# stephane-caron/qpmpc

Measured on AMD Instinct MI355X. Metric: MPC QP builds+solves/sec (batched), higher is better.
Workload: dtype f64

## Files before the change

qpmpc_amd/csrc/mpcqp_quad.hip:

```cpp
#include <hip/hip_runtime.h>
#include <math.h>
#include <stdint.h>
#include <type_traits>

#include "mpcqp.h"
#include "mpcqp_internal.h"
#include "mpcqp_quad_common.h"

namespace mpcqp {

namespace quad {

constexpr int MMAX = 32;
constexpr int MK = 2;

}

using namespace quad;

template <int NX, bool ORD, int WPB, bool SLIM, bool MODEL = false, bool GEN = false>
__global__ void __launch_bounds__(64 * WPB, SLIM ? 2 : 1)
    mpcqp_quad_kernel(const double *__restrict__ gA, const double *__restrict__ gB, const double *__restrict__ gC,
                      const double *__restrict__ ge, const double *__restrict__ gx0, const double *__restrict__ ggoal,
                      const double *__restrict__ gtgt, double *__restrict__ oU, double *__restrict__ olam, int32_t *__restrict__ ostatus,
                      int32_t *__restrict__ oiters, const KernelArgs ka, const int64_t batch)
{
    using T = double;
    extern __shared__ __attribute__((aligned(16))) unsigned char smem_raw[];
    {
        const int64_t b0 = ka.A.batch_stride, b1 = ka.B.batch_stride, b2 = ka.C.batch_stride, b3 = ka.e.batch_stride,
                      b4 = ka.x0.batch_stride, b5 = ka.goal.batch_stride;
        const int64_t s0 = ka.A.step_stride, s1 = ka.B.step_stride, s2 = ka.C.step_stride, s3 = ka.e.step_stride;
        asm volatile("" ::"s"(b0), "s"(b1), "s"(b2), "s"(b3), "s"(b4), "s"(b5), "s"(s0), "s"(s1), "s"(s2), "s"(s3), "s"(ka.N), "s"(ka.nu),
                     "s"(ka.flags), "s"(ka.probe), "s"(gA), "s"(gB), "s"(gC), "s"(ge), "s"(gx0), "s"(ggoal), "s"(ka.n), "s"(ka.m),
                     "s"(batch));
    }
    const int lane = threadIdx.x & 63;
    const int wv = threadIdx.x >> 6;
    const int rb = lane & 48;
    const int l = lane & 15;
    int64_t prob = 4 * ((int64_t)blockIdx.x * WPB + wv) + (rb >> 4);
    const bool valid = prob < batch;
    prob = valid ? prob : batch - 1;
    if constexpr (ORD) {
        const int64_t o = ka.order[prob];
        prob = o < 0 ? 0 : (o >= batch ? batch - 1 : o);
    }
    using CV = Carve<SLIM>;
    constexpr int LDM = CV::LDM, PER = CV::PER;
    T *sm = (T *)smem_raw + (4 * wv + (rb >> 4)) * PER;
    const int n = ka.n, m = ka.m;
    const int row0 = l, row1 = l + NV;
    const bool isc0 = row0 < m, isc1 = row1 < m;
    const T INF = HUGE_VAL;
    constexpr int GS = 33;
    T *Gimg = sm + CV::OFF_M, *Ml = sm + CV::OFF_M;
    T *LTp = sm + CV::OFF_LT + (l * (31 - l)) / 2 - (l + 1);
    T *LTimg = sm + CV::OFF_LT, *Timg = sm + CV::OFF_T, *kAv = sm + CV::OFF_KA;
    int *actv = reinterpret_cast<int *>(sm + CV::OFF_ACT);

    long long *stamp = ka.probe ? (long long *)ka.probe + prob * 16 : nullptr;
    auto tick = [&](int slot) {
        if (stamp && l == 0 && valid) {
            stamp[slot] = (long long)__builtin_readcyclecounter();
            if (slot == 0 || slot == 6) stamp[slot ? 13 : 12] = (long long)__builtin_amdgcn_s_memrealtime();
        }
    };
    tick(0);

    T hval0, hval1;
    bool notpd = false;
    T RM0[NV], RM1[NV], RLt[NV];
    T wv_ = T(0);
    if constexpr (MODEL) {
        const T *model = gA;
        const ModelLayout ml = make_model_layout(ka.nx, ka.N, n, m);
        const int nxr = ka.nx, nT = ka.N * ka.nx;
        const T *x0 = gx0 + prob * ka.x0.batch_stride;
        const T *goal = ggoal ? ggoal + prob * ka.goal.batch_stride : nullptr;
        const T *tgt = gtgt ? gtgt + prob * ka.targets.batch_stride : nullptr;
        notpd = model[ml.total] != T(0);
        {
            T r0[NV], r1[NV];
            ld16(r0, model + ml.off_M + (size_t)(isc0 ? row0 : 0) * NV);
            ld16(r1, model + ml.off_M + (size_t)(isc1 ? row1 : 0) * NV);
            ld16(RLt, model + ml.off_LinvT + (size_t)l * NV);
#pragma unroll
            for (int k = 0; k < NV; ++k) {
                RM0[k] = isc0 ? r0[k] : T(0);
                RM1[k] = isc1 ? r1[k] : T(0);
            }
        }
        auto bound = [&](int row, bool isc) {
            if (!isc) return INF;
            const int mkr = ka.mk, kq = mkr == 2 ? row >> 1 : row / mkr;
            T hh = ge ? ge[prob * ka.e.batch_stride + kq * ka.e.step_stride + (row - kq * mkr)] : model[ml.off_e + row];
            for (int c = 0; c < nxr; ++c) hh -= model[ml.off_Hx + (size_t)row * nxr + c] * x0[c];
            return hh;
        };
        hval0 = bound(row0, isc0);
        hval1 = bound(row1, isc1);
        for (int c = 0; c < nxr; ++c) wv_ += model[ml.off_Wx + (size_t)l * nxr + c] * x0[c];
        if ((ka.flags & MPCQP_Q_TERMINAL) && goal)
            for (int c = 0; c < nxr; ++c) wv_ -= model[ml.off_Wg + (size_t)l * nxr + c] * goal[c];
        if ((ka.flags & MPCQP_Q_STAGE) && tgt)
            for (int j2 = 0; j2 < nT; ++j2) wv_ -= model[ml.off_Wt + (size_t)l * nT + j2] * tgt[j2];
        tick(1);
    } else {
    T Pr[NV];
    T qa;
    T g15a = T(0), g15b = T(0);
    {
        constexpr bool WIDE = GEN && NX > 6;
        const int nx = WIDE ? ka.nx : NX;
        const int nu = ka.nu, N = ka.N;
        constexpr int MKG = GEN ? 4 : MK;
        const int mk = GEN ? ka.mk : MK;
        auto stepof = [&](int row) { return mk == 2 ? row >> 1 : (mk == 1 ? row : (mk == 4 ? row >> 2 : row / 3)); };
        const T *A = gA + prob * ka.A.batch_stride;
        const T *B = gB + prob * ka.B.batch_stride;
        const bool hasC = !GEN || gC != nullptr;
        const T *Cm = hasC ? gC + prob * ka.C.batch_stride : A;
        const T *x0 = gx0 + prob * ka.x0.batch_stride;
        const T *goal = ggoal ? ggoal + prob * ka.goal.batch_stride : nullptr;
        const int sA = ka.A.step_stride ? nx * nx : 0, sB = ka.B.step_stride ? nx * nu : 0, sC = (hasC && ka.C.step_stride) ? mk * nx : 0;
        const bool termP = ka.flags & MPCQP_P_TERMINAL, termQ = (ka.flags & MPCQP_Q_TERMINAL) && goal;
        const T *Dm = (GEN && ka.D.ptr) ? (const T *)ka.D.ptr + prob * ka.D.batch_stride : nullptr;
        const T *tgt = (GEN && gtgt) ? gtgt + prob * ka.targets.batch_stride : nullptr;
        const int sD = (GEN && ka.D.step_stride) ? mk * nu : 0;
        const bool stageP = GEN && (ka.flags & MPCQP_P_STAGE), stageQ = GEN && (ka.flags & MPCQP_Q_STAGE) && tgt;
        constexpr int NAe = NX * NX, NEe = NAe + MKG * NX;
        const int NEr = hasC ? NAe + mk * NX : NAe;
        const bool col = (l < n);
        const int j = col ? (nu == 1 ? l : l / nu) : -1, ii = col ? l - j * nu : 0;
        const int64_t eb = prob * ka.e.batch_stride;
        const int kq0 = stepof(row0), kq1 = stepof(row1);
        const T eval0 = isc0 ? ge[eb + kq0 * ka.e.step_stride + (row0 - kq0 * mk)] : INF;
        const T eval1 = isc1 ? ge[eb + kq1 * ka.e.step_stride + (row1 - kq1 * mk)] : INF;
        const bool xl15 = (l == NV - 1);
        T v[NX], gref[NX], bcol[NX];
#pragma unroll
        for (int s = 0; s < NX; ++s) {
            v[s] = (xl15 && s < nx) ? x0[s < nx ? s : 0] : T(0);
            gref[s] = (termQ && s < nx) ? goal[s < nx ? s : 0] : T(0);
        }
#pragma unroll
        for (int r = 0; r < NX; ++r) bcol[r] = (col && r < nx) ? B[j * sB + (r < nx ? r : 0) * nu + ii] : T(0);
        T dcol[MKG], d15a = T(0), d15b = T(0), tg[NX];
#pragma unroll
        for (int u = 0; u < NX; ++u) tg[u] = T(0);
#pragma unroll
        for (int i2 = 0; i2 < MKG; ++i2) dcol[i2] = T(0);
        if constexpr (GEN) {
            if (Dm) {
#pragma unroll
                for (int i2 = 0; i2 < MKG; ++i2) dcol[i2] = (col && !xl15 && i2 < mk) ? Dm[j * sD + i2 * nu + ii] : T(0);
                if (n == NV) {
                    const int j15 = nu == 1 ? NV - 1 : (NV - 1) / nu, i15 = NV - 1 - j15 * nu;
                    d15a = (isc0 && kq0 == j15) ? Dm[j15 * sD + (row0 - kq0 * mk) * nu + i15] : T(0);
                    d15b = (isc1 && kq1 == j15) ? Dm[j15 * sD + (row1 - kq1 * mk) * nu + i15] : T(0);
                }
            }
            if (stageQ && !WIDE) {
#pragma unroll
                for (int u = 0; u < NX; ++u) tg[u] = (l + 16 * u < N * NX) ? tgt[l + 16 * u] : T(0);
            }
        }
        if constexpr (!WIDE) {
        constexpr int NOP = (NEe + 15) / 16;
        T op[NOP][NV];
        static_for<0, NOP>([&](auto rc) {
            constexpr int r = decltype(rc)::value;
            const int e = l + 16 * r;
            const bool ok = e < NEr;
            const T *p = (e < NAe) ? A + e : Cm + (ok ? e - NAe : 0);
            const int st = (e < NAe) ? sA : sC;
#pragma unroll
            for (int k = 0; k < NV; ++k) {
                const int kc = (k < N) ? k : N - 1;
                op[r][k] = p[kc * st];
            }
        });
        tick(8);
        const T wu = (T)ka.wu;
        qa = T(0);
#pragma unroll
        for (int b = 0; b < NV; ++b) Pr[b] = (l == b) ? (col ? wu : T(1)) : T(0);
        tick(9);
        auto mac = [&](auto idx, auto kc_, T &acc, T xx) {
            constexpr int IDX = decltype(idx)::value, K = decltype(kc_)::value;
            fmac_bcast<IDX % 16>(acc, op[IDX / 16][K], xx);
        };
        static_for<0, NV>([&](auto kk) {
            constexpr int k = decltype(kk)::value;
            if (k < N) {
                if constexpr (!GEN) {
                    T g[MK];
                    static_for<0, MK>([&](auto i2c) {
                        constexpr int i2 = decltype(i2c)::value;
                        T acc = T(0);
                        static_for<0, NX>([&](auto sc) {
                            constexpr int s2 = decltype(sc)::value;
                            mac(ic<NAe + i2 * NX + s2>{}, kk, acc, v[s2]);
                        });
                        g[i2] = acc;
                    });
#pragma unroll
                    for (int i2 = 0; i2 < MK; ++i2) Gimg[l * GS + k * MK + i2] = g[i2];
                } else {
                    static_for<0, MKG>([&](auto i2c) {
                        constexpr int i2 = decltype(i2c)::value;
                        if (i2 < mk) {
                            T acc = T(0);
                            if (hasC) {
                                static_for<0, NX>([&](auto sc) {
                                    constexpr int s2 = decltype(sc)::value;
                                    mac(ic<NAe + i2 * NX + s2>{}, kk, acc, v[s2]);
                                });
                            }
                            acc += (j == k) ? dcol[i2] : T(0);
                            Gimg[l * GS + k * mk + i2] = acc;
                        }
                    });
                }
                if constexpr (GEN && k >= 1) {
                    if (stageP || stageQ) {
                        const T wxs = (T)ka.wx;
                        static_for<0, NX>([&](auto sc) {
                            constexpr int s2 = decltype(sc)::value;
                            constexpr int te = k * NX + s2;
                            T src = xl15 ? T(0) : v[s2];
                            const T t = wxs * src;
                            if (stageQ) qa += t * (row_bcast<NV - 1>(v[s2]) - row_bcast<te % 16>(tg[te / 16]));
                            if (stageP) {
                                dpp_ready(src);
                                static_for<0, NV>([&](auto bc) { fmac_bcast<decltype(bc)::value>(Pr[decltype(bc)::value], src, t); });
                            }
                        });
                    }
                }
                const T hk = (j == k && !xl15) ? T(1) : T(0);
                T w[NX];
                static_for<0, NX>([&](auto rc) {
                    constexpr int r = decltype(rc)::value;
                    T acc = hk * bcol[r];
                    static_for<0, NX>([&](auto sc) {
                        constexpr int s2 = decltype(sc)::value;
                        mac(ic<r * NX + s2>{}, kk, acc, v[s2]);
                    });
                    w[r] = acc;
                });
#pragma unroll
                for (int r = 0; r < NX; ++r) v[r] = w[r];
            }
        });
        } else {
        tick(8);
        const T wu = (T)ka.wu;
        qa = T(0);
#pragma unroll
        for (int b = 0; b < NV; ++b) Pr[b] = (l == b) ? (col ? wu : T(1)) : T(0);
        tick(9);
        constexpr int NAw = NX * NX, NCw = 4 * NX, NEw = NAw + NCw + NX, NOPW = (NEw + 15) / 16;
        T opw[2][NOPW];
        auto fetch = [&](auto dc, int k) {
            constexpr int d = decltype(dc)::value;
            const int kc = k < N ? k : N - 1;
            static_for<0, NOPW>([&](auto rc) {
                constexpr int r = decltype(rc)::value;
                constexpr int e0 = 16 * r;
                const int e = e0 + l;
                T val;
                if constexpr (e0 < NAw) {
                    const int rr = e / NX, ss = e - rr * NX;
                    const bool ok = rr < nx && ss < nx;
                    val = A[kc * sA + (ok ? rr * nx + ss : 0)];
                    val = ok ? val : T(0);
                } else if constexpr (e0 < NAw + NCw) {
                    const int e2 = e - NAw, i2 = e2 / NX, ss = e2 - i2 * NX;
                    const bool ok = hasC && i2 < mk && ss < nx;
                    val = Cm[ok ? kc * sC + i2 * nx + ss : 0];
                    val = ok ? val : T(0);
                } else {
                    const int ss = e - NAw - NCw;
                    const bool ok = stageQ && ss < nx;
                    val = ok ? tgt[kc * nx + ss] : T(0);
                }
                opw[d][r] = val;
            });
        };
        fetch(ic<0>{}, 0);
        fetch(ic<1>{}, 1);
        const T wxs = (T)ka.wx;
        auto cstep = [&](auto dc, int k) {
            constexpr int d = decltype(dc)::value;
            static_for<0, NOPW>([&](auto rc) { dpp_ready(opw[d][decltype(rc)::value]); });
            static_for<0, 4>([&](auto i2c) {
                constexpr int i2 = decltype(i2c)::value;
                if (i2 < mk) {
                    T acc = T(0);
                    if (hasC) {
                        static_for<0, NX>([&](auto sc) {
                            constexpr int s2 = decltype(sc)::value, E = NAw + i2 * NX + s2;
                            fmac_bcast<E % 16>(acc, opw[d][E / 16], v[s2]);
                        });
                    }
                    acc += (j == k) ? dcol[i2] : T(0);
                    Gimg[l * GS + k * mk + i2] = acc;
                }
            });
            if (k >= 1 && (stageP || stageQ)) {
                static_for<0, NX>([&](auto sc) {
                    constexpr int s2 = decltype(sc)::value, E = NAw + NCw + s2;
                    T src = xl15 ? T(0) : v[s2];
                    const T t = wxs * src;
                    if (stageQ) qa += t * (row_bcast<NV - 1>(v[s2]) - row_bcast<E % 16>(opw[d][E / 16]));
                    if (stageP) {
                        dpp_ready(src);
                        static_for<0, NV>([&](auto bc) { fmac_bcast<decltype(bc)::value>(Pr[decltype(bc)::value], src, t); });
                    }
                });
            }
            const T hk = (j == k && !xl15) ? T(1) : T(0);
            T w[NX];
            static_for<0, NX>([&](auto rc) {
                constexpr int r = decltype(rc)::value;
                T acc = hk * bcol[r];
                static_for<0, NX>([&](auto sc) {
                    constexpr int s2 = decltype(sc)::value, E = r * NX + s2;
                    fmac_bcast<E % 16>(acc, opw[d][E / 16], v[s2]);
                });
                w[r] = acc;
            });
#pragma unroll
            for (int r = 0; r < NX; ++r) v[r] = w[r];
            fetch(dc, k + 2);
        };
        for (int k = 0; k < N; k += 2) {
            cstep(ic<0>{}, k);
            if (k + 1 < N) cstep(ic<1>{}, k + 1);
        }
        }
        tick(10);
        const T wt = (T)ka.wt;
        T x[NX];
#pragma unroll
        for (int s = 0; s < NX; ++s) {
            x[s] = row_bcast<NV - 1>(v[s]);
            v[s] = xl15 ? bcol[s] : v[s];
        }
#pragma unroll
        for (int s = 0; s < NX; ++s) {
            const T t = wt * v[s];
            if (termQ) qa += t * (x[s] - gref[s]);
            if (termP) {
                T src = v[s];
                dpp_ready(src);
                static_for<0, NV>([&](auto bc) { fmac_bcast<decltype(bc)::value>(Pr[decltype(bc)::value], src, t); });
            }
        }
        qa = col ? qa : T(0);
        tick(11);
        wave_sync();
        hval0 = isc0 ? eval0 - Gimg[(NV - 1) * GS + row0] : INF;
        hval1 = isc1 ? eval1 - Gimg[(NV - 1) * GS + row1] : INF;
        if constexpr (GEN) {
            g15a = d15a;
            g15b = d15b;
        }
    }
    tick(1);
    {
#pragma unroll
        for (int k = 0; k < NV; ++k) {
            RM0[k] = (isc0 && k < NV - 1) ? Gimg[k * GS + row0] : (GEN && k == NV - 1 ? g15a : T(0));
            RM1[k] = (isc1 && k < NV - 1) ? Gimg[k * GS + row1] : (GEN && k == NV - 1 ? g15b : T(0));
            RLt[k] = (l == k) ? T(1) : T(0);
        }
        static_for<0, NV>([&](auto jc) {
            constexpr int j = decltype(jc)::value;
            const T pij = Pr[j];
            const T piv = row_bcast<j>(pij);
            if (!(piv > T(0))) notpd = true;
            const T rinv = fast_rsqrt(piv);
            const T nt2 = -(pij * rinv * rinv);
            T nl = -(pij * rinv);
            RM0[j] *= rinv;
            RM1[j] *= rinv;
            RLt[j] *= rinv;
            const T wj = qa * rinv;
            wv_ = (l == j) ? wj : wv_;
            {
                T src = pij, wsrc = wj;
                asm volatile("s_nop 1" : "+v"(src), "+v"(nl), "+v"(wsrc) : "v"(RM0[j]), "v"(RM1[j]), "v"(RLt[j]));
                fmac_bcast<j>(qa, wsrc, nl);
                static_for<j + 1, NV>([&](auto kc) {
                    constexpr int k = decltype(kc)::value;
                    fmac_bcast<k>(Pr[k], src, nt2);
                    fmac_bcast<k>(RM0[k], nl, RM0[j]);
                    fmac_bcast<k>(RM1[k], nl, RM1[j]);
                    fmac_bcast<k>(RLt[k], nl, RLt[j]);
                });
            }
        });
        wave_sync();
    }
    }
    tick(2);
    tick(3);
    int status = MPCQP_MAX_ITER, iters = 0;
    T xsol = T(0);
    bool done = notpd;
    bool finished = notpd;
    if (notpd) status = MPCQP_NOT_PD;

    if (isc0) st16(Ml + row0 * LDM, RM0);
    if (isc1) st16(Ml + row1 * LDM, RM1);
    T ltd = T(0);
    if constexpr (SLIM) {
        static_for<0, NV>([&](auto kc) {
            constexpr int k = decltype(kc)::value;
            ltd = (l == k) ? RLt[k] : ltd;
            if (k > l) LTp[k] = RLt[k];
        });
    } else {
        st16(LTimg + l * NV, RLt);
    }
    const T y0 = -wv_;
    T s0, s1, invn0, invn1;
    {
        const T d0 = dot_bcast(wv_, RM0, hval0), d1 = dot_bcast(wv_, RM1, hval1);
        s0 = isc0 ? d0 : INF;
        s1 = isc1 ? d1 : INF;
        const T nn0 = dot16(RM0, RM0), nn1 = dot16(RM1, RM1);
        invn0 = (nn0 > T(0)) ? fast_rsqrt(nn0) : T(1);
        invn1 = (nn1 > T(0)) ? fast_rsqrt(nn1) : T(1);
    }
    const bool sel0 = isc0 && (hval0 < T(1e29)), sel1 = isc1 && (hval1 < T(1e29));
    const T tol = (T)ka.tol;
    const T tolh0 = tol + tol * fabs(hval0), tolh1 = tol + tol * fabs(hval1);
    const int max_iter = ka.max_iter;
    T RT[NV], RH[NV];
#pragma unroll
    for (int k = 0; k < NV; ++k) {
        RT[k] = T(0);
        RH[k] = (l == k) ? T(1) : T(0);
    }
    T lam = T(0);
    int myact = 0;
    bool occ = false;
    bool e0 = sel0, e1 = sel1;
    int nq = 0, p = 0, ldrop = 0;
    unsigned mask = 0;
    bool needp = true, dropping = false;
    T up = T(0);
    int fails = 0;
    T mp[NV];
    auto select = [&]() {
        const bool want = needp & !done & !dropping;
        const unsigned h0 = ~(unsigned)__double2hiint(s0 * invn0), h1 = ~(unsigned)__double2hiint(s1 * invn1);
        const bool v0 = want & e0 & (s0 < -tolh0), v1 = want & e1 & (s1 < -tolh1);
        const unsigned k0 = v0 ? ((h0 & ~31u) | (unsigned)row0) : 0xffffffffu;
        const unsigned k1 = v1 ? ((h1 & ~31u) | (unsigned)row1) : 0xffffffffu;
        const unsigned mkey = row_min(min(k0, k1));
        const bool none = want & (mkey == 0xffffffffu);
        const bool got = want & !none;
        done = done | none;
        status = none ? (int)MPCQP_SOLVED : status;
        p = got ? (int)(mkey & 31u) : p;
        up = got ? T(0) : up;
        needp = needp & !got;
    };
    auto update = [&](auto bc, auto ec, T zn, T cT, T cH) {
        static_for<decltype(bc)::value, decltype(ec)::value>([&](auto kc) {
            constexpr int k = decltype(kc)::value;
            fmac_bcast<k>(RT[k], zn, cT);
            fmac_bcast<k>(RH[k], zn, cH);
        });
    };
#ifndef QUAD_USPLIT
#define QUAD_USPLIT 8
#endif
    constexpr int USPLIT = QUAD_USPLIT;
    T zn = T(0), cT = T(0), cH = T(0);
    wave_sync();
    tick(4);
    for (;;) {
#include "mpcqp_quad_steady.h"
        if (general) for (;;) {
            dpp_ready(zn);
            update(ic<0>{}, ic<USPLIT>{}, zn, cT, cH);
            select();
            ld16(mp, Ml + p * LDM);
            update(ic<USPLIT>{}, ic<NV>{}, zn, cT, cH);
            cT = cH = T(0);
            if (__ballot(!done) == 0ull) break;
            const bool st = !done & !dropping;
            const bool drp = !done & dropping;
            const bool phi = p >= NV;
            const int pl = p & 15;
            const T hd = dot16(RH, mp);
            const T kd0 = dot_bcast(hd, RM0, T(0)), kd1 = dot_bcast(hd, RM1, T(0));
            T inv, t2;
            {
                const T kp = phi ? kd1 : kd0, sq = phi ? s1 : s0, iq = phi ? invn1 : invn0;
                const bool okf = kp * iq * iq > T(DEP_FAST);
                const T iv = fast_rcp(kp);
                inv = row_get(okf ? iv : T(-1), rb, pl);
                t2 = row_get(-sq * iv, rb, pl);
            }
            T rd = dot16(RT, mp);
            pin(rd);
            if (__ballot(st & !(inv > T(0))) != 0ull) {
                T z2 = hd * hd;
                z2 += dpp_mov<ROR8>(z2);
                z2 += dpp_mov<ROR4>(z2);
                z2 += dpp_mov<ROR2>(z2);
                z2 += dpp_mov<ROR1>(z2);
                z2 = row_bcast<0>(z2);
                const T sq = row_get(phi ? s1 : s0, rb, pl), iq = row_get(phi ? invn1 : invn0, rb, pl);
                const bool ok2 = (z2 * iq * iq > T(DEP)) & (z2 > T(0));
                const T iv2 = fast_rcp(z2);
                const bool nearp = !(inv > T(0));
                t2 = nearp ? -sq * iv2 : t2;
                inv = nearp ? (ok2 ? iv2 : T(0)) : inv;
            }
            const bool can_move = (nq < n) & (inv > T(0));
            inv = (can_move & st) ? inv : T(0);
            t2 = can_move ? t2 : INF;
            const int sl = (int)__builtin_ctz(~mask);
            const T r = (occ & st) ? rd : T(0);
            const bool blk = (r > T(0)) & (lam < t2 * r);
            if (__ballot(drp | (st & (!can_move | (iters >= max_iter) | blk))) == 0ull) {
                const T tt = st ? t2 : T(0);
                const bool isnew = st & (l == sl), isp = st & (l == pl);
                iters += st ? 1 : 0;
                zn = hd;
                cT = (l == sl) ? inv : -(r * inv);
                cH = -(hd * inv);
                s0 = fma(tt, kd0, s0);
                s1 = fma(tt, kd1, s1);
                T ln = fma(-tt, r, lam);
                ln = (occ & (ln < T(0))) ? T(0) : ln;
                lam = isnew ? up + tt : ln;
                myact = isnew ? p : myact;
                occ = occ | isnew;
                e0 = e0 & !(isp & !phi);
                e1 = e1 & !(isp & phi);
                mask |= st ? (1u << sl) : 0u;
                nq += st ? 1 : 0;
                needp = needp | st;
                continue;
            }
            bool stepping = st;
            {
                const bool lim = stepping & (iters >= max_iter);
                done = done | lim;
                finished = finished | lim;
                status = lim ? (int)MPCQP_MAX_ITER : status;
                stepping = stepping & !lim;
            }
            iters += stepping ? 1 : 0;
            const bool cand = occ & stepping & (r > T(0));
            T t1 = INF;
            int lq = 0;
            const unsigned long long bl = __ballot(stepping & blk);
            if (bl != 0ull) {
                const T ratio = cand ? lam * fast_rcp(r) : INF;
                unsigned hi, lo;
                ordered(ratio, hi, lo);
                hi = cand ? hi : 0xffffffffu;
                const unsigned mhi = row_min(hi);
                const unsigned k2 = (cand && hi == mhi) ? ((lo & ~31u) | (unsigned)l) : 0xffffffffu;
                const unsigned ml = row_min(k2);
                lq = (int)(ml & 15u);
                const T tl1 = row_get(ratio, rb, lq);
                const bool blocked = ((unsigned)(bl >> rb) & 0xffffu) != 0u;
                t1 = (blocked && mhi != 0xffffffffu) ? tl1 : INF;
            }
            T t = t1 < t2 ? t1 : t2;
            {
                const bool inf = stepping & !(t < INF);
                done = done | inf;
                finished = finished | inf;
                status = inf ? (int)MPCQP_INFEASIBLE : status;
                stepping = stepping & !inf;
            }
            t = stepping ? t : T(0);
            const bool full = stepping & (t2 <= t1);
            zn = hd;
            cT = full ? ((l == sl) ? inv : -(r * inv)) : T(0);
            cH = full ? -(hd * inv) : T(0);
            if (__ballot(drp) != 0ull) {
                T vv[NV];
                T vl = T(0);
                if constexpr (SLIM) {
#pragma unroll
                    for (int k = 0; k < NV; ++k) {
                        vv[k] = row_get(RT[k], rb, ldrop);
                        vl = (l == k) ? vv[k] : vl;
                    }
                } else {
                    ld16(vv, kAv);
                    vl = kAv[l];
                }
                const T tl = dot16(RT, vv);
                const T tld = row_get(tl, rb, ldrop);
                const T itl = fast_rcp(tld);
                if (drp) {
                    zn = vl;
                    cT = (l == ldrop) ? T(-1) : (occ ? -tl * itl : T(0));
                    cH = vl * itl;
                    if (l == ldrop) {
                        lam = T(0);
                        occ = false;
                    }
                    mask &= ~(1u << ldrop);
                    --nq;
                    dropping = false;
                }
            }
            if (stepping) {
                s0 = fma(t, kd0, s0);
                s1 = fma(t, kd1, s1);
                lam -= t * r;
                lam = (occ && lam < T(0)) ? T(0) : lam;
                up += t;
            }
            if (full) {
                if (l == sl) {
                    lam = up;
                    myact = p;
                    occ = true;
                }
                if (l == pl) {
                    e0 = e0 & phi;
                    e1 = e1 & !phi;
                }
                mask |= 1u << sl;
                ++nq;
                needp = true;
            }
            const bool partial = stepping & !full;
            if (__ballot(partial) != 0ull) {
                const int cl = row_get(myact, rb, lq);
                if constexpr (!SLIM) {
                    wave_sync();
                    if (partial && l == lq) st16(kAv, RT);
                }
                if (partial) {
                    if (l == (cl & 15)) {
                        e0 = (cl < NV) ? sel0 : e0;
                        e1 = (cl < NV) ? e1 : sel1;
                    }
                    dropping = true;
                    ldrop = lq;
                }
                if constexpr (!SLIM) wave_sync();
            }
        }
        tick(5);
        if (__ballot(!finished) == 0ull) break;
        int aa[NV];
        if constexpr (SLIM) {
            const int mine = occ ? myact : 0;
            static_for<0, NV>([&](auto ac) { aa[decltype(ac)::value] = __builtin_amdgcn_update_dpp(0, mine, 0x150 + decltype(ac)::value, 0xf, 0xf, false); });
        } else {
            actv[l] = occ ? myact : 0;
            wave_sync();
            const int4 *ap = reinterpret_cast<const int4 *>(actv);
#pragma unroll
            for (int q = 0; q < NV / 4; ++q) {
                const int4 t4 = ap[q];
                aa[4 * q] = t4.x;
                aa[4 * q + 1] = t4.y;
                aa[4 * q + 2] = t4.z;
                aa[4 * q + 3] = t4.w;
            }
        }
        auto ma_dot = [&](T cf) {
            T ma[NV];
#pragma unroll
            for (int a = 0; a < NV; ++a) ma[a] = Ml[aa[a] * LDM + l];
            return dot_bcast(cf, ma, T(0));
        };
        T fresh0, fresh1;
        auto slacks = [&](T yv) {
            const T f0 = dot_bcast(yv, RM0, T(0)), f1 = dot_bcast(yv, RM1, T(0));
            fresh0 = isc0 ? hval0 - f0 : INF;
            fresh1 = isc1 ? hval1 - f1 : INF;
        };
        auto of_act = [&](T x0v, T x1v) {
            const T a = row_get(x0v, rb, myact & 15), b = row_get(x1v, rb, myact & 15);
            return (myact < NV) ? a : b;
        };
        T y = y0 - ma_dot(occ ? lam : T(0));
        slacks(y);
        T rho = of_act(fresh0, fresh1);
        rho = occ ? rho : T(0);
        constexpr double REFTOL = 1e-11;
        const T hact = of_act(hval0, hval1);
        const bool needref = occ & !finished & !(fabs(rho) <= T(REFTOL) * (T(1) + fabs(hact)));
        const unsigned long long nr = __ballot(needref);
        if (nr != 0ull) {
            rho = (((unsigned)(nr >> rb) & 0xffffu) != 0u) ? rho : T(0);
            T uk = T(0);
            if constexpr (SLIM) {
                static_for<0, NV>([&](auto kc) {
                    constexpr int k = decltype(kc)::value;
                    T v = RT[k] * rho;
                    v += dpp_mov<ROR8>(v);
                    v += dpp_mov<ROR4>(v);
                    v += dpp_mov<ROR2>(v);
                    v += dpp_mov<ROR1>(v);
                    uk = (l == k) ? v : uk;
                });
            } else {
                st16(Timg + l * NV, RT);
                wave_sync();
                T tc[NV];
#pragma unroll
                for (int a = 0; a < NV; ++a) tc[a] = Timg[a * NV + l];
                uk = dot_bcast(rho, tc, T(0));
            }
            T dl = -dot_bcast(uk, RT, T(0));
            dl = occ ? dl : T(0);
            if (!finished) {
                const T lraw = lam + dl;
                lam = (occ && lraw < T(0)) ? T(0) : lraw;
            }
            y += uk;
            wave_sync();
            slacks(y);
        }
        bool dirty = row_any((e0 && !(fresh0 >= -T(4) * tolh0)) || (e1 && !(fresh1 >= -T(4) * tolh1)), rb);
        {
            const T ra = of_act(fresh0, fresh1);
            const T ta = of_act(tolh0, tolh1);
            const bool off = row_any(occ && !(fabs(ra) <= T(1e3) * ta), rb);
            const bool neg = row_any(occ && !(lam >= T(0)), rb);
            if (stamp && l == 0 && valid && !finished && done) {
                T worst = T(0);
                stamp[14] = (long long)(dirty ? 1 : 0) | (off ? 2 : 0) | (neg ? 4 : 0) | ((long long)fails << 8) | ((long long)nq << 16);
                (void)worst;
            }
            dirty = dirty || off || neg;
        }
        auto primal = [&]() {
            T lt[NV];
            if constexpr (SLIM) {
                static_for<0, NV>([&](auto kc) {
                    constexpr int k = decltype(kc)::value;
                    lt[k] = (k > l) ? LTp[k > l ? k : l + 1] : ((k == l) ? ltd : T(0));
                });
            } else {
                ld16(lt, LTimg + l * NV);
            }
            return dot_bcast(y, lt, T(0));
        };
        if (!finished && done) {
            if (!dirty) {
                xsol = primal();
                status = MPCQP_SOLVED;
                finished = true;
            } else if (++fails < 4) {
                s0 = fresh0;
                s1 = fresh1;
                status = MPCQP_MAX_ITER;
                done = false;
                needp = true;
            } else {
                xsol = primal();
                status = MPCQP_MAX_ITER;
                finished = true;
            }
        }
        wave_sync();
        if (__ballot(!finished) == 0ull) break;
    }
    tick(6);
    const bool ok = (status == MPCQP_SOLVED);
    T lo0 = T(0), lo1 = T(0);
    if (olam) {
        T *lamv = Ml;
        lamv[row0] = T(0);
        lamv[row1] = T(0);
        wave_sync();
        if (occ) lamv[myact] = lam;
        wave_sync();
        lo0 = ok ? lamv[row0] : T(0);
        lo1 = ok ? lamv[row1] : T(0);
    }
    if (valid) {
        if (l < n) oU[prob * (int64_t)n + l] = ok ? xsol : T(0);
        if (olam) {
            if (isc0) olam[prob * (int64_t)m + row0] = lo0;
            if (isc1) olam[prob * (int64_t)m + row1] = lo1;
        }
        if (l == 0) {
            if (ostatus) ostatus[prob] = status;
            if (oiters) oiters[prob] = iters;
        }
    }
}

[[maybe_unused]] static bool quad_pays(int64_t batch) { return batch > 2 * (int64_t)device_simds_now(); }

static bool quad_general(const KernelArgs &ka)
{
    return ka.nx > 4 || ka.mk != MK || !ka.C.ptr || ka.D.ptr || (ka.flags & (MPCQP_P_STAGE | MPCQP_Q_STAGE));
}

#ifndef MPCQP_QUAD_WIDE_UNIT
bool quad_applies(const KernelArgs &ka)
{
    if (ka.n > NV || ka.m > MMAX || ka.m < 1 || ka.nx < 2 || ka.nx > 16) return false;
    if (ka.mk < 1 || ka.mk > 4 || (!ka.C.ptr && !ka.D.ptr)) return false;
    if (ka.N * ka.mk != ka.m || ka.N > NV) return false;
    if (ka.warm_state || (ka.opt_flags & MPCQP_OPT_SEED_VIOLATED)) return false;
    if (quad_general(ka) && ka.order) return false;
    return true;
}

bool quad_eligible(const KernelArgs &ka, int64_t batch)
{
    if (!quad_applies(ka) || (ka.opt_flags & MPCQP_OPT_TWO_PER_WAVE)) return false;
    return (ka.opt_flags & MPCQP_OPT_FOUR_PER_WAVE) || quad_general(ka) || quad_pays(batch);
}

#endif

template <int NX> static int launch_quad_t(const KernelArgs &ka, int64_t batch, hipStream_t st)
{
    const int64_t waves = (batch + 3) / 4;
    auto go = [&](auto kern, size_t per) {
        const size_t bytes = per * 4 * sizeof(double);
        hipLaunchKernelGGL(kern, dim3((unsigned)waves), dim3(64), bytes, st, (const double *)ka.A.ptr, (const double *)ka.B.ptr,
                           (const double *)ka.C.ptr, (const double *)ka.e.ptr, (const double *)ka.x0.ptr,
                           (const double *)ka.goal.ptr, (const double *)nullptr, (double *)ka.U, (double *)ka.lam, ka.status, ka.iters,
                           ka, batch);
    };
    const bool slim = waves > device_simds_now();
    if (NX > 4 || quad_general(ka)) {
        auto gen = [&](auto kern, size_t per) {
            hipLaunchKernelGGL(kern, dim3((unsigned)waves), dim3(64), per * 4 * sizeof(double), st, (const double *)ka.A.ptr,
                               (const double *)ka.B.ptr, (const double *)ka.C.ptr, (const double *)ka.e.ptr, (const double *)ka.x0.ptr,
                               (const double *)ka.goal.ptr, (const double *)ka.targets.ptr, (double *)ka.U, (double *)ka.lam, ka.status,
                               ka.iters, ka, batch);
        };
        if (slim)
            gen(mpcqp_quad_kernel<NX, false, 1, true, false, true>, Carve<true>::PER);
        else
            gen(mpcqp_quad_kernel<NX, false, 1, false, false, true>, Carve<false>::PER);
    } else if constexpr (NX <= 4) {
        if (ka.order) {
            if (slim)
                go(mpcqp_quad_kernel<NX, true, 1, true>, Carve<true>::PER);
            else
                go(mpcqp_quad_kernel<NX, true, 1, false>, Carve<false>::PER);
        } else if (slim) {
            go(mpcqp_quad_kernel<NX, false, 1, true>, Carve<true>::PER);
        } else {
            go(mpcqp_quad_kernel<NX, false, 1, false>, Carve<false>::PER);
        }
    }
    return (int)hipGetLastError();
}

#ifdef MPCQP_QUAD_WIDE_UNIT
int launch_quad_wide(const KernelArgs &ka, int64_t batch, hipStream_t st)
{
    if (ka.nx == 5) return launch_quad_t<5>(ka, batch, st);
    if (ka.nx == 6) return launch_quad_t<6>(ka, batch, st);
    return ka.nx <= 8 ? launch_quad_t<8>(ka, batch, st) : ka.nx <= 12 ? launch_quad_t<12>(ka, batch, st) : launch_quad_t<16>(ka, batch, st);
}
#else
int launch_quad_wide(const KernelArgs &ka, int64_t batch, hipStream_t st);

int launch_quad(const KernelArgs &ka, int64_t batch, hipStream_t st)
{
    switch (ka.nx) {
    case 2: return launch_quad_t<2>(ka, batch, st);
    case 3: return launch_quad_t<3>(ka, batch, st);
    case 4: return launch_quad_t<4>(ka, batch, st);
    default: return launch_quad_wide(ka, batch, st);
    }
}

bool quad_model_eligible(const KernelArgs &ka, int64_t batch)
{
    if (ka.n > NV || ka.m > MMAX || ka.m < 1 || ka.warm_state || (ka.opt_flags & (MPCQP_OPT_TWO_PER_WAVE | MPCQP_OPT_SEED_VIOLATED)))
        return false;
    return (ka.opt_flags & MPCQP_OPT_FOUR_PER_WAVE) || quad_pays(batch);
}

int launch_quad_model(const KernelArgs &ka, int64_t batch, hipStream_t st)
{
    const int64_t waves = (batch + 3) / 4;
    auto go = [&](auto kern, size_t per) {
        const size_t bytes = per * 4 * sizeof(double);
        hipLaunchKernelGGL(kern, dim3((unsigned)waves), dim3(64), bytes, st, (const double *)ka.model, (const double *)nullptr,
                           (const double *)nullptr, (const double *)ka.e.ptr, (const double *)ka.x0.ptr, (const double *)ka.goal.ptr,
                           (const double *)ka.targets.ptr, (double *)ka.U, (double *)ka.lam, ka.status, ka.iters, ka, batch);
    };
    const bool slim = waves > device_simds_now();
    if (ka.order) {
        if (slim)
            go(mpcqp_quad_kernel<3, true, 1, true, true>, Carve<true>::PER);
        else
            go(mpcqp_quad_kernel<3, true, 1, false, true>, Carve<false>::PER);
    } else if (slim) {
        go(mpcqp_quad_kernel<3, false, 1, true, true>, Carve<true>::PER);
    } else {
        go(mpcqp_quad_kernel<3, false, 1, false, true>, Carve<false>::PER);
    }
    return (int)hipGetLastError();
}

#endif

}
```

qpmpc_amd/csrc/mpcqp_quad_steady.h:

```cpp
bool general = true;
{
    const int iters_in = iters;
    auto maskof = [](bool b) { return (unsigned long long)__builtin_amdgcn_ballot_w64(b); };
    auto lanes = [](unsigned long long m) { return __builtin_amdgcn_inverse_ballot_w64(m); };
    unsigned long long donem = maskof(done), occm = maskof(occ), e0m = maskof(e0), e1m = maskof(e1);
    for (;;) {
        dpp_ready(zn);
        update(ic<0>{}, ic<USPLIT>{}, zn, cT, cH);
        {
            const bool want = !lanes(donem), e0 = lanes(e0m), e1 = lanes(e1m);
            const unsigned h0 = ~(unsigned)__double2hiint(s0 * invn0), h1 = ~(unsigned)__double2hiint(s1 * invn1);
            const bool v0 = want & e0 & (s0 < -tolh0), v1 = want & e1 & (s1 < -tolh1);
            const unsigned k0 = v0 ? ((h0 & ~31u) | (unsigned)row0) : 0xffffffffu;
            const unsigned k1 = v1 ? ((h1 & ~31u) | (unsigned)row1) : 0xffffffffu;
            const unsigned mkey = row_min(min(k0, k1));
            const bool none = want & (mkey == 0xffffffffu);
            donem |= maskof(none);
            status = none ? (int)MPCQP_SOLVED : status;
            p = (want & !none) ? (int)(mkey & 31u) : p;
        }
        ld16(mp, Ml + p * LDM);
        update(ic<USPLIT>{}, ic<NV>{}, zn, cT, cH);
        const bool st = !lanes(donem), occ = lanes(occm);
        if (donem == ~0ull) {
            general = false;
            break;
        }
        const bool phi = p >= NV;
        const int pl = p & 15;
        T hd = dot16(RH, mp);
        T kd0, kd1;
        {
            T a0 = T(0), a1 = T(0), b0 = T(0), b1 = T(0);
            dpp_ready(hd);
            static_for<0, NV / 2>([&](auto kk) {
                constexpr int k = 2 * decltype(kk)::value;
                fmac_bcast<k>(a0, hd, RM0[k]);
                fmac_bcast<k + 1>(a1, hd, RM0[k + 1]);
                fmac_bcast<k>(b0, hd, RM1[k]);
                fmac_bcast<k + 1>(b1, hd, RM1[k + 1]);
            });
            kd0 = a0 + a1;
            kd1 = b0 + b1;
        }
        T inv, t2;
        {
            const T kp = phi ? kd1 : kd0, sq = phi ? s1 : s0, iq = phi ? invn1 : invn0;
            const bool okf = kp * iq * iq > T(DEP_FAST);
            const T iv = fast_rcp(kp);
            inv = row_get(okf ? iv : T(-1), rb, pl);
            t2 = row_get(-sq * iv, rb, pl);
        }
        T rd = dot16(RT, mp);
        pin(rd);
        const bool can_move = (nq < n) & (inv > T(0));
        const int sl = (int)__builtin_ctz(~mask);
        const T r = (occ & st) ? rd : T(0);
        const bool blk = (r > T(0)) & (lam < t2 * r);
        if (maskof(st & (!can_move | (iters >= max_iter) | blk)) != 0ull) break;
        inv = st ? inv : T(0);
        const T tt = st ? t2 : T(0);
        const bool isnew = st & (l == sl), isp = st & (l == pl);
        iters += st ? 1 : 0;
        zn = hd;
        cT = (l == sl) ? inv : -(r * inv);
        cH = -(hd * inv);
        s0 = fma(tt, kd0, s0);
        s1 = fma(tt, kd1, s1);
        T ln = fma(-tt, r, lam);
        ln = (occ & (ln < T(0))) ? T(0) : ln;
        lam = isnew ? tt : ln;
        myact = isnew ? p : myact;
        occm |= maskof(isnew);
        e0m &= ~maskof(isp & !phi);
        e1m &= ~maskof(isp & phi);
        mask |= st ? (1u << sl) : 0u;
        nq += st ? 1 : 0;
    }
    done = lanes(donem);
    occ = lanes(occm);
    e0 = lanes(e0m);
    e1 = lanes(e1m);
    const bool went = iters != iters_in;
    up = (went | !done) ? T(0) : up;
    needp = done ? (needp | went) : false;
    cT = cH = T(0);
}
```

Measured before the change: 207.3 million.

## Fuse constraint drop into partial step and hand off to steady loop

Removes the separate 'dropping' iteration of the general active-set loop. The dual-step drop update is now computed in the same iteration as the partial step, using register row broadcasts (row_get) instead of staging through a shared-memory kAv buffer with wave_syncs. The general loop also restructures so the next-iteration select/update/dot products happen at its tail, and it returns to the faster steady-state loop once no lane needs pricing. Risks include changed control flow and numerics in the drop path, plus extra register pressure from hoisted hd/kd/inv/t2/rd variables.

After: 216.7 million (median of 6 runs). 1.05x the previous value.

```diff
diff --git a/qpmpc_amd/csrc/mpcqp_quad.hip b/qpmpc_amd/csrc/mpcqp_quad.hip
--- a/qpmpc_amd/csrc/mpcqp_quad.hip
+++ b/qpmpc_amd/csrc/mpcqp_quad.hip
@@ -56,7 +56,7 @@
     constexpr int GS = 33;
     T *Gimg = sm + CV::OFF_M, *Ml = sm + CV::OFF_M;
     T *LTp = sm + CV::OFF_LT + (l * (31 - l)) / 2 - (l + 1);
-    T *LTimg = sm + CV::OFF_LT, *Timg = sm + CV::OFF_T, *kAv = sm + CV::OFF_KA;
+    T *LTimg = sm + CV::OFF_LT, *Timg = sm + CV::OFF_T;
     int *actv = reinterpret_cast<int *>(sm + CV::OFF_ACT);
 
     long long *stamp = ka.probe ? (long long *)ka.probe + prob * 16 : nullptr;
@@ -450,14 +450,14 @@
     int myact = 0;
     bool occ = false;
     bool e0 = sel0, e1 = sel1;
-    int nq = 0, p = 0, ldrop = 0;
+    int nq = 0, p = 0;
     unsigned mask = 0;
-    bool needp = true, dropping = false;
+    bool needp = true;
     T up = T(0);
     int fails = 0;
     T mp[NV];
     auto select = [&]() {
-        const bool want = needp & !done & !dropping;
+        const bool want = needp & !done;
         const unsigned h0 = ~(unsigned)__double2hiint(s0 * invn0), h1 = ~(unsigned)__double2hiint(s1 * invn1);
         const bool v0 = want & e0 & (s0 < -tolh0), v1 = want & e1 & (s1 < -tolh1);
         const unsigned k0 = v0 ? ((h0 & ~31u) | (unsigned)row0) : 0xffffffffu;
@@ -483,34 +483,16 @@
 #endif
     constexpr int USPLIT = QUAD_USPLIT;
     T zn = T(0), cT = T(0), cH = T(0);
+    T hd, kd0, kd1, inv, t2, rd;
     wave_sync();
     tick(4);
     for (;;) {
 #include "mpcqp_quad_steady.h"
+        bool resume = false;
         if (general) for (;;) {
-            dpp_ready(zn);
-            update(ic<0>{}, ic<USPLIT>{}, zn, cT, cH);
-            select();
-            ld16(mp, Ml + p * LDM);
-            update(ic<USPLIT>{}, ic<NV>{}, zn, cT, cH);
-            cT = cH = T(0);
-            if (__ballot(!done) == 0ull) break;
-            const bool st = !done & !dropping;
-            const bool drp = !done & dropping;
+            const bool st = !done;
             const bool phi = p >= NV;
             const int pl = p & 15;
-            const T hd = dot16(RH, mp);
-            const T kd0 = dot_bcast(hd, RM0, T(0)), kd1 = dot_bcast(hd, RM1, T(0));
-            T inv, t2;
-            {
-                const T kp = phi ? kd1 : kd0, sq = phi ? s1 : s0, iq = phi ? invn1 : invn0;
-                const bool okf = kp * iq * iq > T(DEP_FAST);
-                const T iv = fast_rcp(kp);
-                inv = row_get(okf ? iv : T(-1), rb, pl);
-                t2 = row_get(-sq * iv, rb, pl);
-            }
-            T rd = dot16(RT, mp);
-            pin(rd);
             if (__ballot(st & !(inv > T(0))) != 0ull) {
                 T z2 = hd * hd;
                 z2 += dpp_mov<ROR8>(z2);
@@ -531,7 +513,7 @@
             const int sl = (int)__builtin_ctz(~mask);
             const T r = (occ & st) ? rd : T(0);
             const bool blk = (r > T(0)) & (lam < t2 * r);
-            if (__ballot(drp | (st & (!can_move | (iters >= max_iter) | blk))) == 0ull) {
+            if (__ballot(st & (!can_move | (iters >= max_iter) | blk)) == 0ull) {
                 const T tt = st ? t2 : T(0);
                 const bool isnew = st & (l == sl), isp = st & (l == pl);
                 iters += st ? 1 : 0;
@@ -550,115 +532,123 @@
                 mask |= st ? (1u << sl) : 0u;
                 nq += st ? 1 : 0;
                 needp = needp | st;
-                continue;
-            }
-            bool stepping = st;
-            {
-                const bool lim = stepping & (iters >= max_iter);
-                done = done | lim;
-                finished = finished | lim;
-                status = lim ? (int)MPCQP_MAX_ITER : status;
-                stepping = stepping & !lim;
-            }
-            iters += stepping ? 1 : 0;
-            const bool cand = occ & stepping & (r > T(0));
-            T t1 = INF;
-            int lq = 0;
-            const unsigned long long bl = __ballot(stepping & blk);
-            if (bl != 0ull) {
-                const T ratio = cand ? lam * fast_rcp(r) : INF;
-                unsigned hi, lo;
-                ordered(ratio, hi, lo);
-                hi = cand ? hi : 0xffffffffu;
-                const unsigned mhi = row_min(hi);
-                const unsigned k2 = (cand && hi == mhi) ? ((lo & ~31u) | (unsigned)l) : 0xffffffffu;
-                const unsigned ml = row_min(k2);
-                lq = (int)(ml & 15u);
-                const T tl1 = row_get(ratio, rb, lq);
-                const bool blocked = ((unsigned)(bl >> rb) & 0xffffu) != 0u;
-                t1 = (blocked && mhi != 0xffffffffu) ? tl1 : INF;
-            }
-            T t = t1 < t2 ? t1 : t2;
-            {
-                const bool inf = stepping & !(t < INF);
-                done = done | inf;
-                finished = finished | inf;
-                status = inf ? (int)MPCQP_INFEASIBLE : status;
-                stepping = stepping & !inf;
-            }
-            t = stepping ? t : T(0);
-            const bool full = stepping & (t2 <= t1);
-            zn = hd;
-            cT = full ? ((l == sl) ? inv : -(r * inv)) : T(0);
-            cH = full ? -(hd * inv) : T(0);
-            if (__ballot(drp) != 0ull) {
-                T vv[NV];
-                T vl = T(0);
-                if constexpr (SLIM) {
-#pragma unroll
-                    for (int k = 0; k < NV; ++k) {
-                        vv[k] = row_get(RT[k], rb, ldrop);
-                        vl = (l == k) ? vv[k] : vl;
+            } else {
+                bool stepping = st;
+                {
+                    const bool lim = stepping & (iters >= max_iter);
+                    done = done | lim;
+                    finished = finished | lim;
+                    status = lim ? (int)MPCQP_MAX_ITER : status;
+                    stepping = stepping & !lim;
+                }
+                iters += stepping ? 1 : 0;
+                const bool cand = occ & stepping & (r > T(0));
+                T t1 = INF;
+                int lq = 0;
+                const unsigned long long bl = __ballot(stepping & blk);
+                if (bl != 0ull) {
+                    const T ratio = cand ? lam * fast_rcp(r) : INF;
+                    unsigned hi, lo;
+                    ordered(ratio, hi, lo);
+                    hi = cand ? hi : 0xffffffffu;
+                    const unsigned mhi = row_min(hi);
+                    const unsigned k2 = (cand && hi == mhi) ? ((lo & ~31u) | (unsigned)l) : 0xffffffffu;
+                    const unsigned ml = row_min(k2);
+                    lq = (int)(ml & 15u);
+                    const T tl1 = row_get(ratio, rb, lq);
+                    const bool blocked = ((unsigned)(bl >> rb) & 0xffffu) != 0u;
+                    t1 = (blocked && mhi != 0xffffffffu) ? tl1 : INF;
+                }
+                T t = t1 < t2 ? t1 : t2;
+                {
+                    const bool inf = stepping & !(t < INF);
+                    done = done | inf;
+                    finished = finished | inf;
+                    status = inf ? (int)MPCQP_INFEASIBLE : status;
+                    stepping = stepping & !inf;
+                }
+                t = stepping ? t : T(0);
+                const bool full = stepping & (t2 <= t1);
+                zn = hd;
+                cT = full ? ((l == sl) ? inv : -(r * inv)) : T(0);
+                cH = full ? -(hd * inv) : T(0);
+                if (stepping) {
+                    s0 = fma(t, kd0, s0);
+                    s1 = fma(t, kd1, s1);
+                    lam -= t * r;
+                    lam = (occ && lam < T(0)) ? T(0) : lam;
+                    up += t;
+                }
+                if (full) {
+                    if (l == sl) {
+                        lam = up;
+                        myact = p;
+                        occ = true;
                     }
-                } else {
-                    ld16(vv, kAv);
-                    vl = kAv[l];
-                }
-                const T tl = dot16(RT, vv);
-                const T tld = row_get(tl, rb, ldrop);
-                const T itl = fast_rcp(tld);
-                if (drp) {
-                    zn = vl;
-                    cT = (l == ldrop) ? T(-1) : (occ ? -tl * itl : T(0));
-                    cH = vl * itl;
-                    if (l == ldrop) {
-                        lam = T(0);
-                        occ = false;
+                    if (l == pl) {
+                        e0 = e0 & phi;
+                        e1 = e1 & !phi;
                     }
-                    mask &= ~(1u << ldrop);
-                    --nq;
-                    dropping = false;
-                }
-            }
-            if (stepping) {
-                s0 = fma(t, kd0, s0);
-                s1 = fma(t, kd1, s1);
-                lam -= t * r;
-                lam = (occ && lam < T(0)) ? T(0) : lam;
-                up += t;
-            }
-            if (full) {
-                if (l == sl) {
-                    lam = up;
-                    myact = p;
-                    occ = true;
-                }
-                if (l == pl) {
-                    e0 = e0 & phi;
-                    e1 = e1 & !phi;
-                }
-                mask |= 1u << sl;
-                ++nq;
-                needp = true;
-            }
-            const bool partial = stepping & !full;
-            if (__ballot(partial) != 0ull) {
-                const int cl = row_get(myact, rb, lq);
-                if constexpr (!SLIM) {
-                    wave_sync();
-                    if (partial && l == lq) st16(kAv, RT);
-                }
-                if (partial) {
-                    if (l == (cl & 15)) {
+                    mask |= 1u << sl;
+                    ++nq;
+                    needp = true;
+                }
+                const bool partial = stepping & !full;
+                if (__ballot(partial) != 0ull) {
+                    const int cl = row_get(myact, rb, lq);
+                    T vl = T(0), ac[4] = {T(0), T(0), T(0), T(0)};
+                    static_for<0, NV / 4>([&](auto cc) {
+                        constexpr int k = 4 * decltype(cc)::value;
+                        T v[4];
+#pragma unroll
+                        for (int j = 0; j < 4; ++j) {
+                            v[j] = row_get(RT[k + j], rb, lq);
+                            vl = (l == k + j) ? v[j] : vl;
+                        }
+#pragma unroll
+                        for (int j = 0; j < 4; ++j) ac[j] = fma(RT[k + j], v[j], ac[j]);
+                        pin(ac[3]);
+                    });
+                    const T tl = (ac[0] + ac[1]) + (ac[2] + ac[3]);
+                    const T tld = row_get(tl, rb, lq);
+                    const T itl = fast_rcp(tld);
+                    if (partial && l == (cl & 15)) {
                         e0 = (cl < NV) ? sel0 : e0;
                         e1 = (cl < NV) ? e1 : sel1;
                     }
-                    dropping = true;
-                    ldrop = lq;
-                }
-                if constexpr (!SLIM) wave_sync();
-            }
-        }
+                    zn = partial ? vl : zn;
+                    cT = partial ? ((l == lq) ? T(-1) : (occ ? -tl * itl : T(0))) : cT;
+                    cH = partial ? vl * itl : cH;
+                    lam = (partial & (l == lq)) ? T(0) : lam;
+                    occ = occ & !(partial & (l == lq));
+                    mask &= partial ? ~(1u << lq) : ~0u;
+                    nq -= partial ? 1 : 0;
+                }
+            }
+            if (__ballot(!done & !needp) == 0ull) {
+                resume = true;
+                break;
+            }
+            dpp_ready(zn);
+            update(ic<0>{}, ic<USPLIT>{}, zn, cT, cH);
+            select();
+            ld16(mp, Ml + p * LDM);
+            update(ic<USPLIT>{}, ic<NV>{}, zn, cT, cH);
+            cT = cH = T(0);
+            hd = dot16(RH, mp);
+            kd0 = dot_bcast(hd, RM0, T(0)), kd1 = dot_bcast(hd, RM1, T(0));
+            {
+                const bool hi = p >= NV;
+                const T kp = hi ? kd1 : kd0, sq = hi ? s1 : s0, iq = hi ? invn1 : invn0;
+                const bool okf = kp * iq * iq > T(DEP_FAST);
+                const T iv = fast_rcp(kp);
+                inv = row_get(okf ? iv : T(-1), rb, p & 15);
+                t2 = row_get(-sq * iv, rb, p & 15);
+            }
+            rd = dot16(RT, mp);
+            pin(rd);
+        }
+        if (resume) continue;
         tick(5);
         if (__ballot(!finished) == 0ull) break;
         int aa[NV];
diff --git a/qpmpc_amd/csrc/mpcqp_quad_steady.h b/qpmpc_amd/csrc/mpcqp_quad_steady.h
--- a/qpmpc_amd/csrc/mpcqp_quad_steady.h
+++ b/qpmpc_amd/csrc/mpcqp_quad_steady.h
@@ -28,8 +28,7 @@
         }
         const bool phi = p >= NV;
         const int pl = p & 15;
-        T hd = dot16(RH, mp);
-        T kd0, kd1;
+        hd = dot16(RH, mp);
         {
             T a0 = T(0), a1 = T(0), b0 = T(0), b1 = T(0);
             dpp_ready(hd);
@@ -43,7 +42,6 @@
             kd0 = a0 + a1;
             kd1 = b0 + b1;
         }
-        T inv, t2;
         {
             const T kp = phi ? kd1 : kd0, sq = phi ? s1 : s0, iq = phi ? invn1 : invn0;
             const bool okf = kp * iq * iq > T(DEP_FAST);
@@ -51,7 +49,7 @@
             inv = row_get(okf ? iv : T(-1), rb, pl);
             t2 = row_get(-sq * iv, rb, pl);
         }
-        T rd = dot16(RT, mp);
+        rd = dot16(RT, mp);
         pin(rd);
         const bool can_move = (nq < n) & (inv > T(0));
         const int sl = (int)__builtin_ctz(~mask);
```
